# GithinjiHans/LZZX-NeRF

Hardware: AMD Instinct MI355X
Metric: rendered samples/s (512x512 triplane head, max_steps 192) (higher is better)
Workload: dtype f32; 1 GPU; cfg3/cfg4 inference: 512x512 frame, max_steps 192, triplane head (3 hash planes + audio/eye cond + SH4), occupancy=ones; step = ray gen + near/far + march/head/composite + blend; rays_per_rank=262144, parallelism=single GPU, mode=fused

## Files before the change

lzzx_nerf_amd/csrc/lz_frame.hip:

```cpp
#include <stdlib.h>

#include <mutex>

#include "lz_march.h"
#include "lz_head_slice.h"
#include "lz_head_f16_slice.h"
#include "lz_head_f16w_slice.h"

#ifndef LZF_WG
#define LZF_WG 1024
#endif
#define LZF_WAVES (LZF_WG / 64)
#define LZF_BINS 256
#define LZF_LUT 256
#define LZF_MARCH_PROBES 2
#define LZF_Q_HEAD 0
#define LZF_Q_SIZE 1
#define LZF_DONE 3
#define LZF_SAMPLES 5
#define LZF_ITER 6
#define LZF_ROWS 72
#define LZF_P_HEAD 8
#define LZF_P_SIZE 9
#define LZF_CEFF 10
// ... 223 lines not shown
        slot[SF_R * ns + sl] = image[(size_t)ray * 3];
        slot[SF_G * ns + sl] = image[(size_t)ray * 3 + 1];
        slot[SF_B * ns + sl] = image[(size_t)ray * 3 + 2];
        slot[SF_A0 * ns + sl] = LZF_OUT(O, amb0_sum)[ray];
        slot[SF_A1 * ns + sl] = LZF_OUT(O, amb1_sum)[ray];
        slot[SF_U * ns + sl] = LZF_OUT(O, unc_sum)[ray];
        sloti[SF_CNT * ns + sl] = (int)LZF_OUT(O, max_steps);
    } else {
#pragma unroll
        for (int f = SF_WS; f <= SF_U; f++) slot[f * ns + sl] = 0.0f;
        sloti[SF_CNT * ns + sl] = 0;
    }
}
enum { LZF_END_BOX = 0, LZF_END_T = 1, LZF_END_CAP = 2 };
__device__ __forceinline__ void lzf_ray_end(const LzfOut& O, bool ph2, int ray, int kind, int composited, int report, float t, float ws, float d,
                                            float r, float g, float b, float a0, float a1, float u) {
    if (__builtin_expect(LZF_OUT(O, cap_mode) != 0, 0)) {
        report = composited;
        if (kind == LZF_END_T) {
            if (LZF_OUT(O, ray_counts)) { report = -composited; LZF_OUT(O, rays_t)[ray] = t; }
            if (!ph2) LZF_OUT(O, ray_last)[ray] = composited - 1;
        } else if (!ph2) {
            LZF_OUT(O, ray_last)[ray] = composited;
            if (kind == LZF_END_CAP) LZF_OUT(O, rays_t)[ray] = t;
        }
    }
    lzf_write_pixel(O, ray, ws, d, r, g, b, a0, a1, u, report);
}

template <int PREC> struct LzfHead;
template <> struct LzfHead<0> {
    using Args = LzHeadArgs; using Ctx = LzHeadCtx; using Out = LzHeadOut;
    static constexpr int LDS_WORDS = LzHeadLds<false>::FLOATS;
    __device__ static __forceinline__ void stage(const Args& P, float* lds, int q, Ctx& c) { lz_head_stage<false>(P, lds, LZF_WG, q, c); }
    __device__ static __forceinline__ LzShPartial sh(const LzfOut& O, const float* slot, int ls, int ns, int q) {
        const int ray = reinterpret_cast<const int*>(slot)[SF_RAY * ns + ls];
        return LzShPartial{ray >= 0 ? LZF_OUT(O, c1sh) + (size_t)ray * LZ_C1_SH_FLOATS + 16 * q : nullptr};
    }
    template <typename ShFn>
    __device__ static __forceinline__ void slice(const Ctx& c, int lane, float x, float y, float z, ShFn f, Out& o) {
        lz_head_slice<false, false, true, true>(c, lane, x, y, z, f, o);
    }
};
template <> struct LzfHead<2> : LzfHead<0> {
    template <typename ShFn>
    __device__ static __forceinline__ void slice(const Ctx& c, int lane, float x, float y, float z, ShFn f, Out& o) {
        lz_head_slice<false, true, true, true>(c, lane, x, y, z, f, o);
    }
};
template <> struct LzfHead<1> {
    using Args = LzHead16Args; using Ctx = LzHead16Ctx; using Out = LzHead16wOut;
    static constexpr int LDS_WORDS = LZ_HEAD16W_LDS_H8 * 4;
    __device__ static __forceinline__ void stage(const Args& P, float* lds, int, Ctx& c) { lz_head16w_stage(P, reinterpret_cast<lz_h8*>(lds), LZF_WG, c); }
    __device__ static __forceinline__ LzShFromSlot16 sh(const LzfOut&, const float* slot, int ls, int ns, int) { return LzShFromSlot16{slot, ls, ns}; }
    template <typename ShFn>
    __device__ static __forceinline__ void slice(const Ctx& c, int lane, float x, float y, float z, ShFn f, Out& o) {
        lz_head16w_slice<true, LZ_F16W_PRIO != 0>(c, lane, x, y, z, f, o);
    }
};

template <int PREC, int S, int ROWS>
__global__ void __launch_bounds__(LZF_WG, LZF_WG / 256)
lz_k_frame(typename LzfHead<PREC>::Args P, LzFrameK F) {
    using HD = LzfHead<PREC>;
    static_assert(PREC == 1 ? ROWS == 2 : (ROWS == 1 || S == 1), "slot rows per wave: f16 two; f32 one, or several with one sample per ray and pass");
    constexpr int NS = 16 * ROWS;
    using FL = LzfFields<PREC, S, ROWS>;
    constexpr int NF = FL::COUNT;
    constexpr int SF_X = FL::X, SF_Y = FL::Y, SF_Z = FL::Z, SF_TS = FL::TS, SF_OSIG = FL::OSIG, SF_OR = FL::OR, SF_OG = FL::OG, SF_OB = FL::OB,
                  SF_OA0 = FL::OA0, SF_OA1 = FL::OA1, SF_OU = FL::OU, SF_IT = FL::IT, SF_RD = FL::RD;
    (void)SF_RD; (void)SF_X; (void)SF_Y; (void)SF_Z; (void)SF_TS; (void)SF_IT; (void)SF_OSIG; (void)SF_OR; (void)SF_OG; (void)SF_OB; (void)SF_OA0; (void)SF_OA1; (void)SF_OU;
    constexpr int SLOT_WORDS = LZF_WAVES * NF * NS;
    __shared__ __align__(16) float lds[HD::LDS_WORDS + SLOT_WORDS + 4 + LZF_LUT];
    const int lane = threadIdx.x & 63, wave = threadIdx.x >> 6;
    const int s = (S > 1) ? (lane & (NS - 1)) : (lane & 15), q = lane >> 4;
    const bool slot_lane = lane < NS;
    static_assert(alignof(typename HD::Args) <= 8, "lz_k_frame(Args P, LzFrameK F): F sits at round8(sizeof(Args)) of the kernel-argument segment");
    const LzfOut OUT = lzf_out<sizeof(typename HD::Args)>();
    const bool ph2 = F.phase2 != 0;
    if (ph2 && F.state[LZF_P_SIZE] <= 0) return;
    typename HD::Ctx ctx;
    HD::stage(P, lds, q, ctx);
    float* slot = lds + HD::LDS_WORDS + wave * NF * NS;
    int* sloti = reinterpret_cast<int*>(slot);
    int* wg_stat = reinterpret_cast<int*>(lds + HD::LDS_WORDS + SLOT_WORDS);
    if (lane < NS) sloti[SF_RAY * NS + lane] = -1;
    if (threadIdx.x < 4) wg_stat[threadIdx.x] = 0;
    uint32_t* mlut = reinterpret_cast<uint32_t*>(lds + HD::LDS_WORDS + SLOT_WORDS + 4);
    const bool use_lut = F.H <= LZF_LUT;
    if (use_lut && threadIdx.x < LZF_LUT) mlut[threadIdx.x] = lz_expand_bits(threadIdx.x);
    __syncthreads();
    const int n_queue = F.state[ph2 ? LZF_P_SIZE : LZF_Q_SIZE];
#define q_head (F.state + (ph2 ? LZF_P_HEAD : LZF_Q_HEAD))
    const int cap = ph2 ? F.state[LZF_CEFF] : (F.cap_mode ? (int)F.max_steps : (((int)F.max_steps + S - 1) / S) * S);
#define cnt_base (ph2 ? (int)F.max_steps : 0)
    constexpr bool KREFILL = ROWS < 3;
#define LZF_RF(name) (KREFILL ? LZF_OUT(OUT, name) : F.name)
    LzMarch m;
    bool dry = n_queue <= 0;
    int my_samples = 0, my_slices = 0;

    if constexpr (S > 1) {
        const int j = s % S, lead = s - j;
        for (;;) {
            if constexpr (PREC != 1 || LZ_F16W_PRIO != 0) __builtin_amdgcn_s_setprio(2);
            const bool leader = slot_lane && j == 0;
            int ray = leader ? sloti[SF_RAY * NS + s] : -1;
            int kk = 0;
            for (int attempt = 0; attempt < 4; attempt++) {
                const bool need = leader && ray < 0 && !dry;
                const unsigned long long mask = __ballot(need);
                if (mask) {
                    const int first = __ffsll((long long)mask) - 1, take = __popcll(mask);
                    int base = 0;
                    if (lane == first) base = atomicAdd(q_head, take);
// ... 82 lines not shown
                            if (more && rank >= 0) {
                                const int sl = lead + rank;
                                slot[SF_X * NS + sl] = cell.x; slot[SF_Y * NS + sl] = cell.y; slot[SF_Z * NS + sl] = cell.z;
                                slot[SF_DT * NS + sl] = cell.dt;
                                slot[SF_TS * NS + sl] = cn;
                            }
                            t0 = t_new;
                            more = more && got < want && t0 < far;
                        }
                        if (leader && grp) {
                            kk = got;
                            if (kk == 0) {
                                const int c0 = sloti[SF_CNT * NS + s];
                                lzf_ray_end(OUT, ph2, ray, LZF_END_BOX, c0, c0, t0, slot[SF_WS * NS + s], slot[SF_D * NS + s], slot[SF_R * NS + s], slot[SF_G * NS + s],
                                            slot[SF_B * NS + s], slot[SF_A0 * NS + s], slot[SF_A1 * NS + s], slot[SF_U * NS + s]);
                                my_samples += c0 - cnt_base;
                                ray = -1;
                                sloti[SF_RAY * NS + s] = -1;
                            }
                        }
                    }
                }
                if (!__ballot(leader && ray < 0 && !dry)) break;
            }
            if (leader) sloti[SF_IT * NS + s] = kk;
            if (!__ballot(kk > 0)) {
                if (dry) break;
                continue;
            }
            const int lkk = sloti[SF_IT * NS + lead];
            const bool live = sloti[SF_RAY * NS + lead] >= 0 && j < lkk;
            const float px = live ? slot[SF_X * NS + s] : 0.0f, py = live ? slot[SF_Y * NS + s] : 0.0f, pz = live ? slot[SF_Z * NS + s] : 0.0f;
            typename HD::Out o;
            HD::slice(ctx, lane, px, py, pz, HD::sh(OUT, slot, lead, NS, q), o);
            my_slices += ROWS;
            if constexpr (PREC == 1) {
                const int hh = lane >> 5;
                slot[(SF_OR + hh) * NS + s] = o.a;
                slot[(hh ? SF_OSIG : SF_OB) * NS + s] = hh ? 1.0f - lz_expf(-o.b * slot[SF_DT * NS + s]) : o.b;
                if (hh == 0) { slot[SF_OA0 * NS + s] = o.ambaud; slot[SF_OA1 * NS + s] = o.eyeatt; slot[SF_OU * NS + s] = o.unc; }
            } else if (q == 0) {
                slot[SF_OSIG * NS + s] = 1.0f - lz_expf(-o.sigma * slot[SF_DT * NS + s]);
                slot[SF_OR * NS + s] = o.rgb[0]; slot[SF_OG * NS + s] = o.rgb[1]; slot[SF_OB * NS + s] = o.rgb[2];
                slot[SF_OA0 * NS + s] = o.ambaud; slot[SF_OA1 * NS + s] = o.eyeatt; slot[SF_OU * NS + s] = o.unc;
            }
            __builtin_amdgcn_wave_barrier();
            if (leader && kk > 0) {
                float ws = slot[SF_WS * NS + s], d = slot[SF_D * NS + s], r = slot[SF_R * NS + s], g = slot[SF_G * NS + s], b = slot[SF_B * NS + s];
                float a0 = slot[SF_A0 * NS + s], a1 = slot[SF_A1 * NS + s], u = slot[SF_U * NS + s], t = slot[SF_T * NS + s];
                int step = 0;
                while (step < kk) {
                    const int sl = s + step;
                    const float alpha = slot[SF_OSIG * NS + sl];
                    const float T = 1 - ws;
                    const float w = alpha * T;
                    ws += w;
                    t = slot[SF_TS * NS + sl];
                    d = lz_fmaf(w, t, d);
                    r = lz_fmaf(w, slot[SF_OR * NS + sl], r);
                    g = lz_fmaf(w, slot[SF_OG * NS + sl], g);
                    b = lz_fmaf(w, slot[SF_OB * NS + sl], b);
                    a0 = a0 + slot[SF_OA0 * NS + sl];
                    a1 = a1 + slot[SF_OA1 * NS + sl];
                    u = lz_fmaf(w, slot[SF_OU * NS + sl], u);
                    if (T < F.T_thresh) break;
                    step++;
                }
// ... 61 lines not shown
                        probes++;
                    }
                    if (have) {
                        slot[SF_T * NS + sl] = t;
                        slot[SF_DT * NS + sl] = dt;
                    } else if (t < far) {
                        slot[SF_T * NS + sl] = t;
                        x = y = z = 0.0f;
                    } else {
                        const int c0 = sloti[SF_CNT * NS + sl];
                        lzf_ray_end(OUT, ph2, ray, LZF_END_BOX, c0, c0, t, slot[SF_WS * NS + sl], slot[SF_D * NS + sl], slot[SF_R * NS + sl], slot[SF_G * NS + sl],
                                    slot[SF_B * NS + sl], slot[SF_A0 * NS + sl], slot[SF_A1 * NS + sl], slot[SF_U * NS + sl]);
                        my_samples += c0 - cnt_base;
                        ray = -1;
                        sloti[SF_RAY * NS + sl] = -1;
                        x = y = z = 0.0f;
                    }
                }
                if (!__ballot(slot_lane && ray < 0 && !dry)) break;
            }
            const unsigned long long have_mask = __ballot(have);
            if (!have_mask) {
                if (dry && !__ballot(slot_lane && ray >= 0)) break;
                continue;
            }
            typename HD::Out o;
            if constexpr (PREC == 1) {
                const int rs = lane & 31, hh = lane >> 5;
                auto lo2 = [](float v) -> float {
                    const auto r = __builtin_amdgcn_permlane32_swap(__float_as_uint(v), __float_as_uint(v), false, false);
                    return __uint_as_float(r[0]);
                };
                const float px = lo2(x), py = lo2(y), pz = lo2(z);
                HD::slice(ctx, lane, px, py, pz, HD::sh(OUT, slot, rs, NS, q), o);
                my_slices += 2;
                slot[(SF_OR + hh) * NS + rs] = o.a;
                slot[(hh ? SF_OSIG : SF_OB) * NS + rs] = o.b;
                if (hh == 0) { slot[SF_OA0 * NS + rs] = o.ambaud; slot[SF_OA1 * NS + rs] = o.eyeatt; slot[SF_OU * NS + rs] = o.unc; }
            } else {
#pragma unroll 1
                for (int row = 0; row < ROWS; row++) {
                    if (ROWS > 1 && !((have_mask >> (16 * row)) & 0xffffull)) continue;
                    const int rs = 16 * row + s;
                    const float px = __shfl(x, rs, 64), py = __shfl(y, rs, 64), pz = __shfl(z, rs, 64);
                    HD::slice(ctx, lane, px, py, pz, HD::sh(OUT, slot, rs, NS, q), o);
                    my_slices++;
                    if (ROWS > 1 && q == 0) {
                        slot[SF_OSIG * NS + rs] = o.sigma;
                        slot[SF_OR * NS + rs] = o.rgb[0]; slot[SF_OG * NS + rs] = o.rgb[1]; slot[SF_OB * NS + rs] = o.rgb[2];
                        slot[SF_OA0 * NS + rs] = o.ambaud; slot[SF_OA1 * NS + rs] = o.eyeatt; slot[SF_OU * NS + rs] = o.unc;
                    }
                }
            }
            __builtin_amdgcn_wave_barrier();
            if (have) {
                float sg, c0, c1, c2, am0, am1, un;
                if constexpr (PREC != 1) { sg = o.sigma; c0 = o.rgb[0]; c1 = o.rgb[1]; c2 = o.rgb[2]; am0 = o.ambaud; am1 = o.eyeatt; un = o.unc; }
                if (ROWS > 1) {
                    sg = slot[SF_OSIG * NS + sl];
                    c0 = slot[SF_OR * NS + sl]; c1 = slot[SF_OG * NS + sl]; c2 = slot[SF_OB * NS + sl];
                    am0 = slot[SF_OA0 * NS + sl]; am1 = slot[SF_OA1 * NS + sl]; un = slot[SF_OU * NS + sl];
                }
                const float dt = slot[SF_DT * NS + sl];
                float ws = slot[SF_WS * NS + sl];
                const float alpha = 1.0f - lz_expf(-sg * dt);
                const float T = 1 - ws;
                const float w = alpha * T;
                ws += w;
                const float t = slot[SF_T * NS + sl] + dt;
                const float d = lz_fmaf(w, t, slot[SF_D * NS + sl]);
                const float r = lz_fmaf(w, c0, slot[SF_R * NS + sl]);
                const float g = lz_fmaf(w, c1, slot[SF_G * NS + sl]);
                const float b = lz_fmaf(w, c2, slot[SF_B * NS + sl]);
                const float a0 = slot[SF_A0 * NS + sl] + am0;
                const float a1 = slot[SF_A1 * NS + sl] + am1;
                const float u = lz_fmaf(w, un, slot[SF_U * NS + sl]);
                const int cnt = sloti[SF_CNT * NS + sl] + 1;
                if (T < F.T_thresh || cnt >= cap) {
// ... 478 lines not shown
```

lzzx_nerf_amd/csrc/lz_head.hip:

```cpp
#include "lz_head_slice.h"

extern "C" uint32_t lz_head_packed_size(void) { return (uint32_t)LZ_HEAD_PACKED_FLOATS; }

__device__ __forceinline__ int lz_chained(int slot, int K) {
    const int t = slot >> 4, r = (slot & 15) >> 2, q = slot & 3;
    const int f = 16 * t + 4 * q + r;
    return f < K ? f : -1;
}

struct LzPackArgs {
    const float* w[LZ_L_COUNT];
    int nout[LZ_L_COUNT];
    int ld[LZ_L_COUNT];
    const float *eye1, *col1, *unc1;
    int has_eye, has_ind;
};

__device__ __forceinline__ int lz_pack_kf(int layer, int slot, const LzPackArgs& a) {
    switch (layer) {
        case LZ_L_A1: case LZ_L_E1: case LZ_L_U1: return slot < 36 ? slot : -1;
        case LZ_L_A2: case LZ_L_S2: case LZ_L_S3: return lz_chained(slot, 64);
        case LZ_L_S1:
            if (slot < 36) return slot;
            if (slot < 68) return 36 + lz_chained(slot - 36, 32);
// ... 78 lines not shown
        if (kf >= 0 && srow >= 0 && a.w[layer]) v = a.w[layer][(size_t)srow * a.ld[layer] + kf];
        packed[(size_t)gid * 4 + j] = (_Float16)v;
    }
}

extern "C" int lz_head_pack_weights_bwd_f16(const float* aud0, const float* aud1, const float* eye0, const float* sig0, const float* sig1,
                                            const float* sig2, const float* col0, int has_eye, int has_ind, void* packed_bwd16,
                                            lz_stream_t stream) {
    LZ_REQUIRE(aud0 && aud1 && sig0 && sig1 && sig2 && col0 && packed_bwd16, LZ_ERR_BAD_ARGUMENT, "head_pack_weights_bwd_f16: null weight");
    LZ_REQUIRE(!has_eye || eye0, LZ_ERR_BAD_ARGUMENT, "head_pack_weights_bwd_f16: eye weights required when has_eye");
    LzPackArgs a;
    const float* w[LZ_L_COUNT] = {aud0, aud1, eye0, sig0, sig1, sig2, col0, nullptr};
    const int nout[LZ_L_COUNT] = {64, 32, 16, 64, 64, 65, 64, 32};
    const int ld[LZ_L_COUNT] = {36, 64, 36, 68 + (has_eye ? 1 : 0), 64, 64, 80 + (has_ind ? 4 : 0), 36};
    for (int i = 0; i < LZ_L_COUNT; i++) { a.w[i] = w[i]; a.nout[i] = nout[i]; a.ld[i] = ld[i]; }
    a.eye1 = a.col1 = a.unc1 = nullptr;
    a.has_eye = has_eye; a.has_ind = has_ind;
    hipLaunchKernelGGL(lz_k_head_pack_bwd_f16, dim3(lz_div_up((uint64_t)LZ_BFRAGS * 64, 256)), dim3(256), 0, lz_st(stream), a,
                       reinterpret_cast<_Float16*>(packed_bwd16));
    LZ_CHECK_LAUNCH("head_pack_weights_bwd_f16");
    return LZ_OK;
}

#define LZ_WG 1024
#define LZ_WG_SAMPLES (LZ_WG / 64 * LZ_T * 16)

__device__ unsigned long long lz_head_probe[2];

template <bool TRAIN_UNC, bool FOLD = false>
__global__ void __launch_bounds__(LZ_WG, LZ_WG / 256)
lz_k_triplane_head(LzHeadArgs P, const float* __restrict__ xyzs, const float* __restrict__ dirs, uint32_t M,
                   const int* __restrict__ count, float* __restrict__ sigmas, float* __restrict__ rgbs,
                   float* __restrict__ amb_aud, float* __restrict__ amb_eye, float* __restrict__ unc_out) {
    __shared__ float wl[LzHeadLds<TRAIN_UNC>::FLOATS];
    uint32_t Meff = M;
    if (count) {
        const int c = *count;
        Meff = c < 0 ? 0u : ((uint32_t)c < M ? (uint32_t)c : M);
    }
    const uint32_t n_slices = (Meff + LZ_T * 16 - 1) / (LZ_T * 16);
    const uint32_t slice_lo = (uint32_t)(((uint64_t)n_slices * blockIdx.x) / gridDim.x);
    const uint32_t slice_hi = (uint32_t)(((uint64_t)n_slices * (blockIdx.x + 1)) / gridDim.x);
    if (slice_lo >= slice_hi) return;
    const bool probe = blockIdx.x == 0 && threadIdx.x == 0;
    unsigned long long probe_c = 0, probe_w = 0;
    if (probe) { probe_c = clock64(); probe_w = wall_clock64(); }

    const int lane = threadIdx.x & 63;
    const int s = lane & 15, q = lane >> 4;
    LzHeadCtx ctx;
    lz_head_stage<TRAIN_UNC>(P, wl, LZ_WG, q, ctx);
    __syncthreads();

    int* queue = reinterpret_cast<int*>(wl + LzHeadLds<TRAIN_UNC>::TAB) + LZ_LVTAB_QUEUE;
    for (;;) {
        int slice = 0;
        if (lane == 0) slice = atomicAdd(queue, 1);
        slice = __builtin_amdgcn_readfirstlane(slice);
        if (slice_lo + (uint32_t)slice >= slice_hi) {
            if (probe) { lz_head_probe[0] = clock64() - probe_c; lz_head_probe[1] = wall_clock64() - probe_w; }
            break;
        }
        const uint32_t base = (slice_lo + (uint32_t)slice) * (LZ_T * 16);
        uint32_t m = base + s;
        if (m >= Meff) m = Meff - 1;
        const float px = xyzs[(size_t)m * 3], py = xyzs[(size_t)m * 3 + 1], pz = xyzs[(size_t)m * 3 + 2];
        LzHeadOut o;
        lz_head_slice<TRAIN_UNC, FOLD>(ctx, lane, px, py, pz,
                                 lz_sh_from_dir([&](float& dx, float& dy, float& dz) { dx = dirs[(size_t)m * 3]; dy = dirs[(size_t)m * 3 + 1]; dz = dirs[(size_t)m * 3 + 2]; }), o);
        if (q == 0 && base + s < Meff) {
            sigmas[m] = o.sigma;
            rgbs[(size_t)m * 3] = o.rgb[0]; rgbs[(size_t)m * 3 + 1] = o.rgb[1]; rgbs[(size_t)m * 3 + 2] = o.rgb[2];
            amb_aud[m] = o.ambaud;
            if (amb_eye) amb_eye[m] = o.eyeatt;
            unc_out[m] = o.unc;
        }
    }
}

int lz_head_forward_f16_impl(const lz_head_params* p, const float* xyzs, const float* dirs, uint32_t M, const int32_t* count, float* sigmas,
                             float* rgbs, float* amb_aud, float* amb_eye, float* unc, hipStream_t st);

extern "C" int lz_debug_head_clocks(uint64_t* out2) {
    LZ_REQUIRE(out2, LZ_ERR_BAD_ARGUMENT, "debug_head_clocks: null");
// ... 44 lines not shown
```

lzzx_nerf_amd/csrc/lz_head_layers.h:

```cpp
#ifndef LZ_HEAD_LAYERS_H
#define LZ_HEAD_LAYERS_H
#include "lz_common.h"
#include "lzzx_detmath.h"

typedef float lz_f4 __attribute__((ext_vector_type(4)));

enum { LZ_L_A1 = 0, LZ_L_A2, LZ_L_E1, LZ_L_S1, LZ_L_S2, LZ_L_S3, LZ_L_C1, LZ_L_U1, LZ_L_COUNT };
constexpr int LZ_KS[LZ_L_COUNT] = {   9, 16,  9, 18, 16, 16, 21,  9 };
constexpr int LZ_NT[LZ_L_COUNT] = {   4,  2,  1,  4,  4,  4,  4,  2 };
constexpr int lz_frag_base(int layer) {
    int b = 0;
    for (int i = 0; i < layer; i++) b += LZ_KS[i] * LZ_NT[i];
    return b;
}
constexpr int lz_kt(int layer) { return (LZ_KS[layer] + 3) / 4; }
constexpr int lz_bfrag_base(int layer) {
    int b = 0;
    for (int i = 0; i < layer; i++) b += i == LZ_L_U1 ? 0 : lz_kt(i) * LZ_NT[i];
    return b;
}
constexpr int LZ_BFRAGS = lz_bfrag_base(LZ_L_COUNT);
constexpr int LZ_FRAGS_INFER = lz_frag_base(LZ_L_U1);
constexpr int LZ_FRAGS_ALL = lz_frag_base(LZ_L_COUNT);
constexpr int LZ_WV_C2 = 0, LZ_WV_SIG = 192, LZ_WV_E2 = 256, LZ_WV_U2 = 272, LZ_WV_FLOATS = 320;
static_assert(LZ_FRAGS_ALL * 64 + LZ_WV_FLOATS == LZ_HEAD_PACKED_FLOATS, "packed size mismatch with the header");


struct LzHeadArgs {
    const float* emb[3];
    const int* offsets;
    const float* packed;
    const float* enc_a;
    const float* ind_code;
    const float* eye;
    float bound;
    float scale[12];
    uint32_t res[12];
    int testing;
};

template <int LAYER, int T, int K0, int K1>
__device__ __forceinline__ void lz_layer_ks(const float* __restrict__ wl, int lane, const float (&b)[T][LZ_KS[LAYER]],
                                            lz_f4 (&acc)[LZ_NT[LAYER]][T]) {
    constexpr int NT = LZ_NT[LAYER];
    static_assert(0 <= K0 && K0 <= K1 && K1 <= LZ_KS[LAYER], "k-step range");
    const float* frag = wl + lz_frag_base(LAYER) * 64 + lane;
#pragma unroll
    for (int ks = K0; ks < K1; ks++) {
        float a[NT];
#pragma unroll
        for (int ft = 0; ft < NT; ft++) a[ft] = frag[(ks * NT + ft) * 64];
#pragma unroll
        for (int ft = 0; ft < NT; ft++)
#pragma unroll
            for (int j = 0; j < T; j++) acc[ft][j] = __builtin_amdgcn_mfma_f32_16x16x4f32(a[ft], b[j][ks], acc[ft][j], 0, 0, 0);
    }
}
template <int LAYER, int T>
__device__ __forceinline__ void lz_layer(const float* __restrict__ wl, int lane, const float (&b)[T][LZ_KS[LAYER]],
                                         lz_f4 (&acc)[LZ_NT[LAYER]][T]) {
    lz_layer_ks<LAYER, T, 0, LZ_KS[LAYER]>(wl, lane, b, acc);
}

__device__ __forceinline__ float lz_relu(float v) { return v > 0.0f ? v : 0.0f; }

template <int NTILE>
__device__ __forceinline__ float lz_lane_dot(const float* __restrict__ wrow, int q, const float (&x)[4 * NTILE]) {
    float acc = 0.0f;
#pragma unroll
    for (int t = 0; t < NTILE; t++)
#pragma unroll
        for (int r = 0; r < 4; r++) acc = lz_fmaf(wrow[16 * t + 4 * q + r], x[4 * t + r], acc);
    acc += __shfl_xor(acc, 16, 64);
    acc += __shfl_xor(acc, 32, 64);
    return acc;
}

#endif
```

lzzx_nerf_amd/csrc/lz_head_slice.h:

```cpp
#ifndef LZ_HEAD_SLICE_H
#define LZ_HEAD_SLICE_H
#include "lz_common.h"
#include "lzzx_detmath.h"
#include "lzzx_sh_eval.h"
#include "lz_head_gather.h"
#include "lz_head_layers.h"

#define LZ_T 1

struct LzHeadCtx {
    const float* wl;
    const int* tab;
    const float* lenca;
    const float* emb[3];
    float bound, two_bound, eye_v, indq;
    const float* lind;
    bool has_eye, has_ind;
};

struct LzHeadOut {
    float sigma, rgb[3], ambaud, eyeatt, unc;
};

template <bool TRAIN_UNC>
struct LzHeadLds {
    static constexpr int NFRAG = TRAIN_UNC ? LZ_FRAGS_ALL : LZ_FRAGS_INFER;
    static constexpr int WV = NFRAG * 64, TAB = WV + LZ_WV_FLOATS, FLOATS = TAB + LZ_LVTAB_WORDS;
};

template <bool TRAIN_UNC>
__device__ __forceinline__ void lz_head_stage(const LzHeadArgs& P, float* wl, uint32_t n_threads, int q, LzHeadCtx& hc) {
    using L = LzHeadLds<TRAIN_UNC>;
    const float4* src = reinterpret_cast<const float4*>(P.packed);
    float4* dst = reinterpret_cast<float4*>(wl);
    for (uint32_t i = threadIdx.x; i < (uint32_t)L::NFRAG * 16; i += n_threads) dst[i] = src[i];
    if (threadIdx.x < LZ_WV_FLOATS) wl[L::WV + threadIdx.x] = P.packed[LZ_FRAGS_ALL * 64 + threadIdx.x];
    int* tab = reinterpret_cast<int*>(wl + L::TAB);
    lz_level_table_fill(tab, P.offsets, P.scale, P.res);
    if (threadIdx.x < 32) wl[L::TAB + LZ_LVTAB_ENCA + threadIdx.x] = P.enc_a[threadIdx.x];
    hc.wl = wl;
    hc.tab = tab;
    hc.lenca = wl + L::TAB + LZ_LVTAB_ENCA;
    hc.emb[0] = P.emb[0]; hc.emb[1] = P.emb[1]; hc.emb[2] = P.emb[2];
    hc.bound = P.bound;
    hc.two_bound = 2.0f * P.bound;
    hc.has_eye = P.eye != nullptr;
    hc.eye_v = hc.has_eye ? P.eye[0] : 0.0f;
    hc.indq = P.ind_code ? P.ind_code[q] : 0.0f;
    hc.has_ind = P.ind_code != nullptr;
    if (threadIdx.x < 4) wl[L::TAB + LZ_LVTAB_IND + threadIdx.x] = P.ind_code ? P.ind_code[threadIdx.x] : 0.0f;
    hc.lind = wl + L::TAB + LZ_LVTAB_IND;
}

template <typename DirFn>
struct LzShFromDir {
    DirFn dirfn;
    float o[16];
    static constexpr bool C1_PARTIAL = false;
    __device__ __forceinline__ explicit LzShFromDir(DirFn f) : dirfn(f) {}
    __device__ __forceinline__ void issue(int) {}
    __device__ __forceinline__ void prepare() {
        float dx, dy, dz;
        dirfn(dx, dy, dz);
        lz_sh_eval(dx, dy, dz, 4, o, nullptr, nullptr, nullptr);
    }
    __device__ __forceinline__ float comp_iq(int i, int q) const {
        return q == 0 ? o[4 * i] : (q == 1 ? o[4 * i + 1] : (q == 2 ? o[4 * i + 2] : o[4 * i + 3]));
    }
    __device__ __forceinline__ float comp_qj(int q, int j) const {
        return q == 0 ? o[j] : (q == 1 ? o[4 + j] : (q == 2 ? o[8 + j] : o[12 + j]));
    }
};
template <typename DirFn>
__device__ __forceinline__ LzShFromDir<DirFn> lz_sh_from_dir(DirFn f) { return LzShFromDir<DirFn>(f); }

constexpr int LZ_C1_SH_KS = 4;
constexpr int LZ_C1_SH_FLOATS = 64;
template <typename ShFn>
__device__ __forceinline__ void lz_c1_sh_partial(const float* __restrict__ wl, int lane, ShFn& sh, lz_f4 (&acc)[4][1]) {
    const int q = lane >> 4;
    float b[1][LZ_KS[LZ_L_C1]];
    sh.prepare();
#pragma unroll
    for (int i = 0; i < LZ_KS[LZ_L_C1]; i++) b[0][i] = i < LZ_C1_SH_KS ? sh.comp_iq(i, q) : 0.0f;
#pragma unroll
    for (int ft = 0; ft < 4; ft++) acc[ft][0] = lz_f4{0, 0, 0, 0};
    lz_layer_ks<LZ_L_C1, 1, 0, LZ_C1_SH_KS>(wl, lane, b, acc);
}
struct LzShPartial {
    static constexpr bool C1_PARTIAL = true;
    const float* row;
    lz_f4 p[4];
    __device__ __forceinline__ void issue(int) {
#pragma unroll
        for (int ft = 0; ft < 4; ft++) p[ft] = row ? *reinterpret_cast<const lz_f4*>(row + 4 * ft) : lz_f4{0, 0, 0, 0};
    }
    __device__ __forceinline__ lz_f4 part(int ft) const { return p[ft]; }
};

template <bool TRAIN_UNC, bool FOLD = false, bool IN_RANGE = false, bool YIELD = false, typename ShFn>
__device__ __forceinline__ void lz_head_slice(const LzHeadCtx& hc, int lane, float px, float py, float pz, ShFn shfn, LzHeadOut& out) {
    static_assert(!(TRAIN_UNC && FOLD), "the folded colour net is an inference arrangement");
    constexpr int WV = LzHeadLds<TRAIN_UNC>::WV;
    const int q = lane >> 4;
    float encx[LZ_T][9];
    lz_head_gather<IN_RANGE, LZ_GATHER_PACK32, YIELD, true>(hc.emb, hc.tab, px, py, pz, q, hc.bound, hc.two_bound, encx[0]);
    __builtin_amdgcn_sched_barrier(0);

    float att[LZ_T][8];
    {
        lz_f4 acc1[4][LZ_T];
#pragma unroll
        for (int ft = 0; ft < 4; ft++)
#pragma unroll
            for (int j = 0; j < LZ_T; j++) acc1[ft][j] = lz_f4{0, 0, 0, 0};
        lz_layer<LZ_L_A1, LZ_T>(hc.wl, lane, encx, acc1);
        float b2[LZ_T][16];
#pragma unroll
        for (int j = 0; j < LZ_T; j++)
#pragma unroll
            for (int ft = 0; ft < 4; ft++)
#pragma unroll
                for (int r = 0; r < 4; r++) b2[j][4 * ft + r] = lz_relu(acc1[ft][j][r]);
        lz_f4 acc2[2][LZ_T];
#pragma unroll
        for (int ft = 0; ft < 2; ft++)
#pragma unroll
            for (int j = 0; j < LZ_T; j++) acc2[ft][j] = lz_f4{0, 0, 0, 0};
        lz_layer<LZ_L_A2, LZ_T>(hc.wl, lane, b2, acc2);
#pragma unroll
        for (int j = 0; j < LZ_T; j++)
#pragma unroll
            for (int ft = 0; ft < 2; ft++)
#pragma unroll
                for (int r = 0; r < 4; r++) att[j][4 * ft + r] = acc2[ft][j][r];
    }
    float ambaud[LZ_T];
#pragma unroll
    for (int j = 0; j < LZ_T; j++) {
        float acc = 0.0f;
#pragma unroll
        for (int k = 0; k < 8; k++) acc = lz_fmaf(att[j][k], att[j][k], acc);
        acc += __shfl_xor(acc, 16, 64);
        acc += __shfl_xor(acc, 32, 64);
        ambaud[j] = sqrtf(acc);
    }
    float eyeatt[LZ_T];
#pragma unroll
    for (int j = 0; j < LZ_T; j++) eyeatt[j] = 0.0f;
    if (hc.has_eye) {
        lz_f4 acce[1][LZ_T];
#pragma unroll
        for (int j = 0; j < LZ_T; j++) acce[0][j] = lz_f4{0, 0, 0, 0};
        lz_layer<LZ_L_E1, LZ_T>(hc.wl, lane, encx, acce);
        float be[LZ_T][4];
#pragma unroll
        for (int j = 0; j < LZ_T; j++)
#pragma unroll
            for (int r = 0; r < 4; r++) be[j][r] = lz_relu(acce[0][j][r]);
#pragma unroll
        for (int j = 0; j < LZ_T; j++) eyeatt[j] = lz_sigmoidf(lz_lane_dot<1>(hc.wl + WV + LZ_WV_E2, q, be[j]));
    }
    float uncv[LZ_T];
    if constexpr (TRAIN_UNC) {
        lz_f4 accu[2][LZ_T];
#pragma unroll
        for (int ft = 0; ft < 2; ft++)
#pragma unroll
            for (int j = 0; j < LZ_T; j++) accu[ft][j] = lz_f4{0, 0, 0, 0};
        lz_layer<LZ_L_U1, LZ_T>(hc.wl, lane, encx, accu);
        float bu[LZ_T][8];
#pragma unroll
        for (int j = 0; j < LZ_T; j++)
#pragma unroll
            for (int ft = 0; ft < 2; ft++)
#pragma unroll
                for (int r = 0; r < 4; r++) bu[j][4 * ft + r] = lz_relu(accu[ft][j][r]);
#pragma unroll
        for (int j = 0; j < LZ_T; j++) uncv[j] = lz_softplusf(lz_lane_dot<2>(hc.wl + WV + LZ_WV_U2, q, bu[j]));
    } else {
#pragma unroll
        for (int j = 0; j < LZ_T; j++) uncv[j] = lz_softplusf(0.0f);
    }
    float geo[LZ_T][16];
    float sig_pre[LZ_T];
    {
        float b1[LZ_T][18];
#pragma unroll
        for (int j = 0; j < LZ_T; j++) {
#pragma unroll
            for (int i = 0; i < 9; i++) b1[j][i] = encx[j][i];
#pragma unroll
            for (int t = 0; t < 2; t++)
#pragma unroll
                for (int r = 0; r < 4; r++) b1[j][9 + 4 * t + r] = hc.lenca[16 * t + 4 * q + r] * att[j][4 * t + r];
            b1[j][17] = 0.0f;
        }
        lz_f4 acc1[4][LZ_T];
#pragma unroll
        for (int ft = 0; ft < 4; ft++)
#pragma unroll
            for (int j = 0; j < LZ_T; j++) acc1[ft][j] = lz_f4{0, 0, 0, 0};
        lz_layer_ks<LZ_L_S1, LZ_T, 0, 17>(hc.wl, lane, b1, acc1);
        if (hc.has_eye) {
            const float* w68 = hc.wl + (lz_frag_base(LZ_L_S1) + 17 * LZ_NT[LZ_L_S1]) * 64 + 4 * q;
#pragma unroll
            for (int j = 0; j < LZ_T; j++) {
                const float e = hc.eye_v * eyeatt[j];
#pragma unroll
                for (int ft = 0; ft < 4; ft++) {
                    const lz_f4 w = *reinterpret_cast<const lz_f4*>(w68 + 64 * ft);
#pragma unroll
                    for (int r = 0; r < 4; r++) acc1[ft][j][r] = lz_fmaf(w[r], e, acc1[ft][j][r]);
                }
            }
        }
        float b2[LZ_T][16];
#pragma unroll
        for (int j = 0; j < LZ_T; j++)
#pragma unroll
            for (int ft = 0; ft < 4; ft++)
#pragma unroll
                for (int r = 0; r < 4; r++) b2[j][4 * ft + r] = lz_relu(acc1[ft][j][r]);
        shfn.issue(q);
        lz_f4 acc2[4][LZ_T];
#pragma unroll
        for (int ft = 0; ft < 4; ft++)
#pragma unroll
            for (int j = 0; j < LZ_T; j++) acc2[ft][j] = lz_f4{0, 0, 0, 0};
        lz_layer<LZ_L_S2, LZ_T>(hc.wl, lane, b2, acc2);
        float b3[LZ_T][16];
#pragma unroll
        for (int j = 0; j < LZ_T; j++)
#pragma unroll
            for (int ft = 0; ft < 4; ft++)
#pragma unroll
                for (int r = 0; r < 4; r++) b3[j][4 * ft + r] = lz_relu(acc2[ft][j][r]);
        if constexpr (FOLD) {
#pragma unroll
            for (int j = 0; j < LZ_T; j++)
#pragma unroll
                for (int k = 0; k < 16; k++) geo[j][k] = b3[j][k];
        } else {
            lz_f4 acc3[4][LZ_T];
#pragma unroll
            for (int ft = 0; ft < 4; ft++)
#pragma unroll
                for (int j = 0; j < LZ_T; j++) acc3[ft][j] = lz_f4{0, 0, 0, 0};
            lz_layer<LZ_L_S3, LZ_T>(hc.wl, lane, b3, acc3);
#pragma unroll
            for (int j = 0; j < LZ_T; j++)
#pragma unroll
                for (int ft = 0; ft < 4; ft++)
#pragma unroll
                    for (int r = 0; r < 4; r++) geo[j][4 * ft + r] = acc3[ft][j][r];
        }
#pragma unroll
        for (int j = 0; j < LZ_T; j++) sig_pre[j] = lz_lane_dot<4>(hc.wl + WV + LZ_WV_SIG, q, b3[j]);
    }
    float rgb[LZ_T][3];
    {
        constexpr bool IND_VALU = !FOLD;
        float b1[LZ_T][21];
        lz_f4 acc1[4][LZ_T];
#pragma unroll
        for (int j = 0; j < LZ_T; j++) {
            if constexpr (ShFn::C1_PARTIAL) {
#pragma unroll
                for (int i = 0; i < LZ_C1_SH_KS; i++) b1[j][i] = 0.0f;
#pragma unroll
                for (int ft = 0; ft < 4; ft++) acc1[ft][j] = shfn.part(ft);
            } else {
                shfn.prepare();
#pragma unroll
                for (int i = 0; i < 4; i++) b1[j][i] = shfn.comp_iq(i, q);
#pragma unroll
                for (int ft = 0; ft < 4; ft++) acc1[ft][j] = lz_f4{0, 0, 0, 0};
            }
#pragma unroll
            for (int k = 0; k < 16; k++) b1[j][4 + k] = geo[j][k];
            b1[j][20] = IND_VALU ? 0.0f : hc.indq;
        }
        lz_layer_ks<LZ_L_C1, LZ_T, ShFn::C1_PARTIAL ? LZ_C1_SH_KS : 0, LZ_KS[LZ_L_C1] - (IND_VALU ? 1 : 0)>(hc.wl, lane, b1, acc1);
        if (IND_VALU && hc.has_ind) {
            const float* w80 = hc.wl + (lz_frag_base(LZ_L_C1) + 20 * LZ_NT[LZ_L_C1]) * 64 + 4 * q;
            const lz_f4 ind = *reinterpret_cast<const lz_f4*>(hc.lind);
#pragma unroll
            for (int j = 0; j < LZ_T; j++)
#pragma unroll
                for (int k = 0; k < 4; k++)
#pragma unroll
                    for (int ft = 0; ft < 4; ft++) {
                        const lz_f4 w = *reinterpret_cast<const lz_f4*>(w80 + 64 * ft + 16 * k);
#pragma unroll
                        for (int r = 0; r < 4; r++) acc1[ft][j][r] = lz_fmaf(w[r], ind[k], acc1[ft][j][r]);
                    }
        }
        float b2[LZ_T][16];
#pragma unroll
        for (int j = 0; j < LZ_T; j++)
#pragma unroll
            for (int ft = 0; ft < 4; ft++)
#pragma unroll
                for (int r = 0; r < 4; r++) b2[j][4 * ft + r] = lz_relu(acc1[ft][j][r]);
#pragma unroll
        for (int j = 0; j < LZ_T; j++) {
            float d[3];
#pragma unroll
            for (int c = 0; c < 3; c++) d[c] = lz_lane_dot<4>(hc.wl + WV + LZ_WV_C2 + 64 * c, q, b2[j]);
            const float arg = q == 0 ? -d[0] : (q == 1 ? -d[1] : (q == 2 ? -d[2] : sig_pre[j]));
            const float e = lz_expf(arg);
            const float v = q == 3 ? e : (1.0f / (1.0f + e)) * 1.002f - 0.001f;
            const int s0 = lane & 15;
#pragma unroll
            for (int c = 0; c < 3; c++) rgb[j][c] = __shfl(v, s0 + 16 * c, 64);
            sig_pre[j] = __shfl(v, s0 + 48, 64);
        }
    }
    out.sigma = sig_pre[0];
    out.rgb[0] = rgb[0][0]; out.rgb[1] = rgb[0][1]; out.rgb[2] = rgb[0][2];
    out.ambaud = ambaud[0];
    out.eyeatt = eyeatt[0];
    out.unc = uncv[0];
}
#endif
```

Baseline: 2.799 billion samples/s.

## Stage head weights k-step-major in LDS and prefetch next MFMA fragment

Adds a k-step-major LDS weight layout so each lane pulls all NT output-tile weights for one k-step with a single vector load. A new layer routine prefetches the next k-step (or the first fragment of the next layer) while the current MFMAs issue, with scheduling barriers to interleave LDS reads and MFMAs. The frame kernel uses this for the S==1 refill paths and the standalone head kernel always does. The per-step path keeps the planar layout. The cost is extra live registers and a more complex staging transpose, which may lower occupancy.

```diff
diff --git a/lzzx_nerf_amd/csrc/lz_frame.hip b/lzzx_nerf_amd/csrc/lz_frame.hip
--- a/lzzx_nerf_amd/csrc/lz_frame.hip
+++ b/lzzx_nerf_amd/csrc/lz_frame.hip
@@ -279,28 +279,32 @@
 template <> struct LzfHead<0> {
     using Args = LzHeadArgs; using Ctx = LzHeadCtx; using Out = LzHeadOut;
     static constexpr int LDS_WORDS = LzHeadLds<false>::FLOATS;
-    __device__ static __forceinline__ void stage(const Args& P, float* lds, int q, Ctx& c) { lz_head_stage<false>(P, lds, LZF_WG, q, c); }
+    template <bool KSMAJOR>
+    __device__ static __forceinline__ void stage(const Args& P, float* lds, int q, Ctx& c) {
+        lz_head_stage<false, KSMAJOR ? LZ_W_KSMAJOR : LZ_W_PLANAR>(P, lds, LZF_WG, q, c);
+    }
     __device__ static __forceinline__ LzShPartial sh(const LzfOut& O, const float* slot, int ls, int ns, int q) {
         const int ray = reinterpret_cast<const int*>(slot)[SF_RAY * ns + ls];
         return LzShPartial{ray >= 0 ? LZF_OUT(O, c1sh) + (size_t)ray * LZ_C1_SH_FLOATS + 16 * q : nullptr};
     }
-    template <typename ShFn>
+    template <bool AHEAD, typename ShFn>
     __device__ static __forceinline__ void slice(const Ctx& c, int lane, float x, float y, float z, ShFn f, Out& o) {
-        lz_head_slice<false, false, true, true>(c, lane, x, y, z, f, o);
+        lz_head_slice<false, false, true, true, AHEAD>(c, lane, x, y, z, f, o);
     }
 };
 template <> struct LzfHead<2> : LzfHead<0> {
-    template <typename ShFn>
+    template <bool AHEAD, typename ShFn>
     __device__ static __forceinline__ void slice(const Ctx& c, int lane, float x, float y, float z, ShFn f, Out& o) {
-        lz_head_slice<false, true, true, true>(c, lane, x, y, z, f, o);
+        lz_head_slice<false, true, true, true, AHEAD>(c, lane, x, y, z, f, o);
     }
 };
 template <> struct LzfHead<1> {
     using Args = LzHead16Args; using Ctx = LzHead16Ctx; using Out = LzHead16wOut;
     static constexpr int LDS_WORDS = LZ_HEAD16W_LDS_H8 * 4;
+    template <bool>
     __device__ static __forceinline__ void stage(const Args& P, float* lds, int, Ctx& c) { lz_head16w_stage(P, reinterpret_cast<lz_h8*>(lds), LZF_WG, c); }
     __device__ static __forceinline__ LzShFromSlot16 sh(const LzfOut&, const float* slot, int ls, int ns, int) { return LzShFromSlot16{slot, ls, ns}; }
-    template <typename ShFn>
+    template <bool, typename ShFn>
     __device__ static __forceinline__ void slice(const Ctx& c, int lane, float x, float y, float z, ShFn f, Out& o) {
         lz_head16w_slice<true, LZ_F16W_PRIO != 0>(c, lane, x, y, z, f, o);
     }
@@ -327,7 +331,7 @@
     const bool ph2 = F.phase2 != 0;
     if (ph2 && F.state[LZF_P_SIZE] <= 0) return;
     typename HD::Ctx ctx;
-    HD::stage(P, lds, q, ctx);
+    HD::template stage<S == 1>(P, lds, q, ctx);
     float* slot = lds + HD::LDS_WORDS + wave * NF * NS;
     int* sloti = reinterpret_cast<int*>(slot);
     int* wg_stat = reinterpret_cast<int*>(lds + HD::LDS_WORDS + SLOT_WORDS);
@@ -476,7 +480,7 @@
             const bool live = sloti[SF_RAY * NS + lead] >= 0 && j < lkk;
             const float px = live ? slot[SF_X * NS + s] : 0.0f, py = live ? slot[SF_Y * NS + s] : 0.0f, pz = live ? slot[SF_Z * NS + s] : 0.0f;
             typename HD::Out o;
-            HD::slice(ctx, lane, px, py, pz, HD::sh(OUT, slot, lead, NS, q), o);
+            HD::template slice<false>(ctx, lane, px, py, pz, HD::sh(OUT, slot, lead, NS, q), o);
             my_slices += ROWS;
             if constexpr (PREC == 1) {
                 const int hh = lane >> 5;
@@ -604,7 +608,7 @@
                     return __uint_as_float(r[0]);
                 };
                 const float px = lo2(x), py = lo2(y), pz = lo2(z);
-                HD::slice(ctx, lane, px, py, pz, HD::sh(OUT, slot, rs, NS, q), o);
+                HD::template slice<true>(ctx, lane, px, py, pz, HD::sh(OUT, slot, rs, NS, q), o);
                 my_slices += 2;
                 slot[(SF_OR + hh) * NS + rs] = o.a;
                 slot[(hh ? SF_OSIG : SF_OB) * NS + rs] = o.b;
@@ -615,7 +619,7 @@
                     if (ROWS > 1 && !((have_mask >> (16 * row)) & 0xffffull)) continue;
                     const int rs = 16 * row + s;
                     const float px = __shfl(x, rs, 64), py = __shfl(y, rs, 64), pz = __shfl(z, rs, 64);
-                    HD::slice(ctx, lane, px, py, pz, HD::sh(OUT, slot, rs, NS, q), o);
+                    HD::template slice<true>(ctx, lane, px, py, pz, HD::sh(OUT, slot, rs, NS, q), o);
                     my_slices++;
                     if (ROWS > 1 && q == 0) {
                         slot[SF_OSIG * NS + rs] = o.sigma;
diff --git a/lzzx_nerf_amd/csrc/lz_head.hip b/lzzx_nerf_amd/csrc/lz_head.hip
--- a/lzzx_nerf_amd/csrc/lz_head.hip
+++ b/lzzx_nerf_amd/csrc/lz_head.hip
@@ -134,7 +134,7 @@
 lz_k_triplane_head(LzHeadArgs P, const float* __restrict__ xyzs, const float* __restrict__ dirs, uint32_t M,
                    const int* __restrict__ count, float* __restrict__ sigmas, float* __restrict__ rgbs,
                    float* __restrict__ amb_aud, float* __restrict__ amb_eye, float* __restrict__ unc_out) {
-    __shared__ float wl[LzHeadLds<TRAIN_UNC>::FLOATS];
+    __shared__ __align__(16) float wl[LzHeadLds<TRAIN_UNC>::FLOATS];
     uint32_t Meff = M;
     if (count) {
         const int c = *count;
@@ -151,7 +151,7 @@
     const int lane = threadIdx.x & 63;
     const int s = lane & 15, q = lane >> 4;
     LzHeadCtx ctx;
-    lz_head_stage<TRAIN_UNC>(P, wl, LZ_WG, q, ctx);
+    lz_head_stage<TRAIN_UNC, LZ_W_KSMAJOR>(P, wl, LZ_WG, q, ctx);
     __syncthreads();
 
     int* queue = reinterpret_cast<int*>(wl + LzHeadLds<TRAIN_UNC>::TAB) + LZ_LVTAB_QUEUE;
diff --git a/lzzx_nerf_amd/csrc/lz_head_layers.h b/lzzx_nerf_amd/csrc/lz_head_layers.h
--- a/lzzx_nerf_amd/csrc/lz_head_layers.h
+++ b/lzzx_nerf_amd/csrc/lz_head_layers.h
@@ -39,7 +39,28 @@
     int testing;
 };
 
-template <int LAYER, int T, int K0, int K1>
+enum { LZ_W_PLANAR = 0, LZ_W_KSMAJOR = 1 };
+template <int LAYER>
+__device__ __forceinline__ constexpr int lz_w_at(int ks, int lane, int ft) {
+    return (lz_frag_base(LAYER) + ks * LZ_NT[LAYER]) * 64 + lane * LZ_NT[LAYER] + ft;
+}
+template <int NT> struct LzWFrag { float v[NT]; };
+template <int LAYER>
+__device__ __forceinline__ LzWFrag<LZ_NT[LAYER]> lz_wfetch(const float* __restrict__ wl, int lane, int ks) {
+    constexpr int NT = LZ_NT[LAYER];
+    LzWFrag<NT> a;
+    if constexpr (NT > 1) {
+        typedef float vec_t __attribute__((ext_vector_type(NT)));
+        const vec_t w = *reinterpret_cast<const vec_t*>(wl + lz_w_at<LAYER>(ks, lane, 0));
+#pragma unroll
+        for (int ft = 0; ft < NT; ft++) a.v[ft] = w[ft];
+    } else {
+        a.v[0] = wl[lz_w_at<LAYER>(ks, lane, 0)];
+    }
+    return a;
+}
+
+template <int LAYER, int T, int K0, int K1, int LAYOUT = LZ_W_PLANAR>
 __device__ __forceinline__ void lz_layer_ks(const float* __restrict__ wl, int lane, const float (&b)[T][LZ_KS[LAYER]],
                                             lz_f4 (&acc)[LZ_NT[LAYER]][T]) {
     constexpr int NT = LZ_NT[LAYER];
@@ -48,13 +69,51 @@
 #pragma unroll
     for (int ks = K0; ks < K1; ks++) {
         float a[NT];
+        if constexpr (LAYOUT == LZ_W_KSMAJOR) {
+            const LzWFrag<NT> w = lz_wfetch<LAYER>(wl, lane, ks);
 #pragma unroll
-        for (int ft = 0; ft < NT; ft++) a[ft] = frag[(ks * NT + ft) * 64];
+            for (int ft = 0; ft < NT; ft++) a[ft] = w.v[ft];
+        } else {
+#pragma unroll
+            for (int ft = 0; ft < NT; ft++) a[ft] = frag[(ks * NT + ft) * 64];
+        }
 #pragma unroll
         for (int ft = 0; ft < NT; ft++)
 #pragma unroll
             for (int j = 0; j < T; j++) acc[ft][j] = __builtin_amdgcn_mfma_f32_16x16x4f32(a[ft], b[j][ks], acc[ft][j], 0, 0, 0);
     }
+}
+constexpr int lz_nt_or1(int layer) { return layer < 0 ? 1 : LZ_NT[layer]; }
+template <bool AHEAD, int LAYER, int T, int K0, int K1, int NEXT = -1, int NEXT_K = 0, int NEXT2 = -1, int NEXT2_K = 0>
+__device__ __forceinline__ LzWFrag<lz_nt_or1(NEXT)> lz_layer_ks_ahead(const float* __restrict__ wl, int lane, const float (&b)[T][LZ_KS[LAYER]],
+                                                                     lz_f4 (&acc)[LZ_NT[LAYER]][T], LzWFrag<LZ_NT[LAYER]> a,
+                                                                     LzWFrag<lz_nt_or1(NEXT2)>* next2 = nullptr) {
+    constexpr int NT = LZ_NT[LAYER];
+    static_assert(0 <= K0 && K0 < K1 && K1 <= LZ_KS[LAYER], "k-step range");
+    LzWFrag<lz_nt_or1(NEXT)> next = {};
+    if constexpr (!AHEAD) {
+        lz_layer_ks<LAYER, T, K0, K1, LZ_W_PLANAR>(wl, lane, b, acc);
+        return next;
+    }
+#pragma unroll
+    for (int ks = K0; ks < K1; ks++) {
+        LzWFrag<NT> ahead = a;
+        if (ks + 1 < K1) ahead = lz_wfetch<LAYER>(wl, lane, ks + 1);
+        else {
+            if constexpr (NEXT >= 0) next = lz_wfetch<NEXT>(wl, lane, NEXT_K);
+            if constexpr (NEXT2 >= 0) *next2 = lz_wfetch<NEXT2>(wl, lane, NEXT2_K);
+        }
+#pragma unroll
+        for (int ft = 0; ft < NT; ft++)
+#pragma unroll
+            for (int j = 0; j < T; j++) acc[ft][j] = __builtin_amdgcn_mfma_f32_16x16x4f32(a.v[ft], b[j][ks], acc[ft][j], 0, 0, 0);
+        if (ks + 1 < K1 || NEXT >= 0) __builtin_amdgcn_sched_group_barrier(0x100 , 1, 0);
+        if (ks + 1 == K1 && NEXT2 >= 0) __builtin_amdgcn_sched_group_barrier(0x100, 1, 0);
+        __builtin_amdgcn_sched_group_barrier(0x8 , NT * T, 0);
+        a = ahead;
+    }
+    __builtin_amdgcn_sched_barrier(0);
+    return next;
 }
 template <int LAYER, int T>
 __device__ __forceinline__ void lz_layer(const float* __restrict__ wl, int lane, const float (&b)[T][LZ_KS[LAYER]],
diff --git a/lzzx_nerf_amd/csrc/lz_head_slice.h b/lzzx_nerf_amd/csrc/lz_head_slice.h
--- a/lzzx_nerf_amd/csrc/lz_head_slice.h
+++ b/lzzx_nerf_amd/csrc/lz_head_slice.h
@@ -28,12 +28,35 @@
     static constexpr int WV = NFRAG * 64, TAB = WV + LZ_WV_FLOATS, FLOATS = TAB + LZ_LVTAB_WORDS;
 };
 
-template <bool TRAIN_UNC>
+template <int LAYER>
+__device__ __forceinline__ void lz_head_stage_ksmajor(const float* __restrict__ packed, float* wl, uint32_t n_threads) {
+    constexpr int NT = LZ_NT[LAYER], BASE = lz_frag_base(LAYER);
+    const float4* src = reinterpret_cast<const float4*>(packed) + BASE * 16;
+    for (uint32_t i = threadIdx.x; i < (uint32_t)(LZ_KS[LAYER] * NT * 16); i += n_threads) {
+        const float4 v = src[i];
+        const int f = (int)(i >> 4), l0 = (int)(i & 15) * 4;
+        float* d = wl + lz_w_at<LAYER>(f / NT, l0, f % NT);
+        d[0] = v.x; d[NT] = v.y; d[2 * NT] = v.z; d[3 * NT] = v.w;
+    }
+}
+template <bool TRAIN_UNC, int LAYER = 0>
+__device__ __forceinline__ void lz_head_stage_ksmajor_all(const float* __restrict__ packed, float* wl, uint32_t n_threads) {
+    if constexpr (LAYER < (TRAIN_UNC ? LZ_L_COUNT : LZ_L_U1)) {
+        lz_head_stage_ksmajor<LAYER>(packed, wl, n_threads);
+        lz_head_stage_ksmajor_all<TRAIN_UNC, LAYER + 1>(packed, wl, n_threads);
+    }
+}
+
+template <bool TRAIN_UNC, int LAYOUT = LZ_W_PLANAR>
 __device__ __forceinline__ void lz_head_stage(const LzHeadArgs& P, float* wl, uint32_t n_threads, int q, LzHeadCtx& hc) {
     using L = LzHeadLds<TRAIN_UNC>;
-    const float4* src = reinterpret_cast<const float4*>(P.packed);
-    float4* dst = reinterpret_cast<float4*>(wl);
-    for (uint32_t i = threadIdx.x; i < (uint32_t)L::NFRAG * 16; i += n_threads) dst[i] = src[i];
+    if constexpr (LAYOUT == LZ_W_KSMAJOR) {
+        lz_head_stage_ksmajor_all<TRAIN_UNC>(P.packed, wl, n_threads);
+    } else {
+        const float4* src = reinterpret_cast<const float4*>(P.packed);
+        float4* dst = reinterpret_cast<float4*>(wl);
+        for (uint32_t i = threadIdx.x; i < (uint32_t)L::NFRAG * 16; i += n_threads) dst[i] = src[i];
+    }
     if (threadIdx.x < LZ_WV_FLOATS) wl[L::WV + threadIdx.x] = P.packed[LZ_FRAGS_ALL * 64 + threadIdx.x];
     int* tab = reinterpret_cast<int*>(wl + L::TAB);
     lz_level_table_fill(tab, P.offsets, P.scale, P.res);
@@ -98,23 +121,27 @@
     __device__ __forceinline__ lz_f4 part(int ft) const { return p[ft]; }
 };
 
-template <bool TRAIN_UNC, bool FOLD = false, bool IN_RANGE = false, bool YIELD = false, typename ShFn>
+template <bool TRAIN_UNC, bool FOLD = false, bool IN_RANGE = false, bool YIELD = false, bool AHEAD = true, typename ShFn>
 __device__ __forceinline__ void lz_head_slice(const LzHeadCtx& hc, int lane, float px, float py, float pz, ShFn shfn, LzHeadOut& out) {
     static_assert(!(TRAIN_UNC && FOLD), "the folded colour net is an inference arrangement");
     constexpr int WV = LzHeadLds<TRAIN_UNC>::WV;
     const int q = lane >> 4;
     float encx[LZ_T][9];
     lz_head_gather<IN_RANGE, LZ_GATHER_PACK32, YIELD, true>(hc.emb, hc.tab, px, py, pz, q, hc.bound, hc.two_bound, encx[0]);
+    LzWFrag<4> w_a1 = {};
+    if constexpr (AHEAD) w_a1 = lz_wfetch<LZ_L_A1>(hc.wl, lane, 0);
     __builtin_amdgcn_sched_barrier(0);
 
     float att[LZ_T][8];
+    LzWFrag<1> w_e1;
+    LzWFrag<4> w_s1;
     {
         lz_f4 acc1[4][LZ_T];
 #pragma unroll
         for (int ft = 0; ft < 4; ft++)
 #pragma unroll
             for (int j = 0; j < LZ_T; j++) acc1[ft][j] = lz_f4{0, 0, 0, 0};
-        lz_layer<LZ_L_A1, LZ_T>(hc.wl, lane, encx, acc1);
+        const LzWFrag<2> w_a2 = lz_layer_ks_ahead<AHEAD, LZ_L_A1, LZ_T, 0, LZ_KS[LZ_L_A1], LZ_L_A2, 0>(hc.wl, lane, encx, acc1, w_a1);
         float b2[LZ_T][16];
 #pragma unroll
         for (int j = 0; j < LZ_T; j++)
@@ -127,7 +154,7 @@
         for (int ft = 0; ft < 2; ft++)
 #pragma unroll
             for (int j = 0; j < LZ_T; j++) acc2[ft][j] = lz_f4{0, 0, 0, 0};
-        lz_layer<LZ_L_A2, LZ_T>(hc.wl, lane, b2, acc2);
+        w_e1 = lz_layer_ks_ahead<AHEAD, LZ_L_A2, LZ_T, 0, LZ_KS[LZ_L_A2], LZ_L_E1, 0, LZ_L_S1, 0>(hc.wl, lane, b2, acc2, w_a2, &w_s1);
 #pragma unroll
         for (int j = 0; j < LZ_T; j++)
 #pragma unroll
@@ -148,11 +175,12 @@
     float eyeatt[LZ_T];
 #pragma unroll
     for (int j = 0; j < LZ_T; j++) eyeatt[j] = 0.0f;
+    if constexpr (AHEAD) asm volatile("" : "+v"(w_e1.v[0]));
     if (hc.has_eye) {
         lz_f4 acce[1][LZ_T];
 #pragma unroll
         for (int j = 0; j < LZ_T; j++) acce[0][j] = lz_f4{0, 0, 0, 0};
-        lz_layer<LZ_L_E1, LZ_T>(hc.wl, lane, encx, acce);
+        lz_layer_ks_ahead<AHEAD, LZ_L_E1, LZ_T, 0, LZ_KS[LZ_L_E1]>(hc.wl, lane, encx, acce, w_e1);
         float be[LZ_T][4];
 #pragma unroll
         for (int j = 0; j < LZ_T; j++)
@@ -168,7 +196,7 @@
         for (int ft = 0; ft < 2; ft++)
 #pragma unroll
             for (int j = 0; j < LZ_T; j++) accu[ft][j] = lz_f4{0, 0, 0, 0};
-        lz_layer<LZ_L_U1, LZ_T>(hc.wl, lane, encx, accu);
+        lz_layer_ks_ahead<AHEAD, LZ_L_U1, LZ_T, 0, LZ_KS[LZ_L_U1]>(hc.wl, lane, encx, accu, lz_wfetch<LZ_L_U1>(hc.wl, lane, 0));
         float bu[LZ_T][8];
 #pragma unroll
         for (int j = 0; j < LZ_T; j++)
@@ -184,6 +212,7 @@
     }
     float geo[LZ_T][16];
     float sig_pre[LZ_T];
+    LzWFrag<4> w_c1;
     {
         float b1[LZ_T][18];
 #pragma unroll
@@ -201,17 +230,21 @@
         for (int ft = 0; ft < 4; ft++)
 #pragma unroll
             for (int j = 0; j < LZ_T; j++) acc1[ft][j] = lz_f4{0, 0, 0, 0};
-        lz_layer_ks<LZ_L_S1, LZ_T, 0, 17>(hc.wl, lane, b1, acc1);
+        if constexpr (AHEAD) __builtin_amdgcn_sched_barrier(0);
+        const LzWFrag<4> w_s2 = lz_layer_ks_ahead<AHEAD, LZ_L_S1, LZ_T, 0, 17, LZ_L_S2, 0>(hc.wl, lane, b1, acc1, w_s1);
         if (hc.has_eye) {
-            const float* w68 = hc.wl + (lz_frag_base(LZ_L_S1) + 17 * LZ_NT[LZ_L_S1]) * 64 + 4 * q;
+            const float* w68 = AHEAD ? hc.wl + lz_w_at<LZ_L_S1>(17, 4 * q, 0) : hc.wl + (lz_frag_base(LZ_L_S1) + 17 * LZ_NT[LZ_L_S1]) * 64 + 4 * q;
 #pragma unroll
             for (int j = 0; j < LZ_T; j++) {
                 const float e = hc.eye_v * eyeatt[j];
 #pragma unroll
-                for (int ft = 0; ft < 4; ft++) {
-                    const lz_f4 w = *reinterpret_cast<const lz_f4*>(w68 + 64 * ft);
-#pragma unroll
-                    for (int r = 0; r < 4; r++) acc1[ft][j][r] = lz_fmaf(w[r], e, acc1[ft][j][r]);
+                for (int u = 0; u < 4; u++) {
+                    const lz_f4 w = *reinterpret_cast<const lz_f4*>(w68 + (AHEAD ? 4 : 64) * u);
+#pragma unroll
+                    for (int v = 0; v < 4; v++) {
+                        const int ft = AHEAD ? v : u, r = AHEAD ? u : v;
+                        acc1[ft][j][r] = lz_fmaf(w[v], e, acc1[ft][j][r]);
+                    }
                 }
             }
         }
@@ -228,7 +261,8 @@
         for (int ft = 0; ft < 4; ft++)
 #pragma unroll
             for (int j = 0; j < LZ_T; j++) acc2[ft][j] = lz_f4{0, 0, 0, 0};
-        lz_layer<LZ_L_S2, LZ_T>(hc.wl, lane, b2, acc2);
+        constexpr int C1_K0 = ShFn::C1_PARTIAL ? LZ_C1_SH_KS : 0;
+        const LzWFrag<4> w_s3 = lz_layer_ks_ahead<AHEAD, LZ_L_S2, LZ_T, 0, LZ_KS[LZ_L_S2], FOLD ? LZ_L_C1 : LZ_L_S3, FOLD ? C1_K0 : 0>(hc.wl, lane, b2, acc2, w_s2);
         float b3[LZ_T][16];
 #pragma unroll
         for (int j = 0; j < LZ_T; j++)
@@ -241,13 +275,14 @@
             for (int j = 0; j < LZ_T; j++)
 #pragma unroll
                 for (int k = 0; k < 16; k++) geo[j][k] = b3[j][k];
+            w_c1 = w_s3;
         } else {
             lz_f4 acc3[4][LZ_T];
 #pragma unroll
             for (int ft = 0; ft < 4; ft++)
 #pragma unroll
                 for (int j = 0; j < LZ_T; j++) acc3[ft][j] = lz_f4{0, 0, 0, 0};
-            lz_layer<LZ_L_S3, LZ_T>(hc.wl, lane, b3, acc3);
+            w_c1 = lz_layer_ks_ahead<AHEAD, LZ_L_S3, LZ_T, 0, LZ_KS[LZ_L_S3], LZ_L_C1, C1_K0>(hc.wl, lane, b3, acc3, w_s3);
 #pragma unroll
             for (int j = 0; j < LZ_T; j++)
 #pragma unroll
@@ -281,19 +316,23 @@
             for (int k = 0; k < 16; k++) b1[j][4 + k] = geo[j][k];
             b1[j][20] = IND_VALU ? 0.0f : hc.indq;
         }
-        lz_layer_ks<LZ_L_C1, LZ_T, ShFn::C1_PARTIAL ? LZ_C1_SH_KS : 0, LZ_KS[LZ_L_C1] - (IND_VALU ? 1 : 0)>(hc.wl, lane, b1, acc1);
+        if constexpr (AHEAD) __builtin_amdgcn_sched_barrier(0);
+        lz_layer_ks_ahead<AHEAD, LZ_L_C1, LZ_T, ShFn::C1_PARTIAL ? LZ_C1_SH_KS : 0, LZ_KS[LZ_L_C1] - (IND_VALU ? 1 : 0)>(hc.wl, lane, b1, acc1, w_c1);
         if (IND_VALU && hc.has_ind) {
-            const float* w80 = hc.wl + (lz_frag_base(LZ_L_C1) + 20 * LZ_NT[LZ_L_C1]) * 64 + 4 * q;
+            const float* w80 = AHEAD ? hc.wl + lz_w_at<LZ_L_C1>(20, 4 * q, 0) : hc.wl + (lz_frag_base(LZ_L_C1) + 20 * LZ_NT[LZ_L_C1]) * 64 + 4 * q;
             const lz_f4 ind = *reinterpret_cast<const lz_f4*>(hc.lind);
 #pragma unroll
             for (int j = 0; j < LZ_T; j++)
 #pragma unroll
                 for (int k = 0; k < 4; k++)
 #pragma unroll
-                    for (int ft = 0; ft < 4; ft++) {
-                        const lz_f4 w = *reinterpret_cast<const lz_f4*>(w80 + 64 * ft + 16 * k);
-#pragma unroll
-                        for (int r = 0; r < 4; r++) acc1[ft][j][r] = lz_fmaf(w[r], ind[k], acc1[ft][j][r]);
+                    for (int u = 0; u < 4; u++) {
+                        const lz_f4 w = *reinterpret_cast<const lz_f4*>(w80 + (AHEAD ? 64 * k + 4 * u : 64 * u + 16 * k));
+#pragma unroll
+                        for (int v = 0; v < 4; v++) {
+                            const int ft = AHEAD ? v : u, r = AHEAD ? u : v;
+                            acc1[ft][j][r] = lz_fmaf(w[v], ind[k], acc1[ft][j][r]);
+                        }
                     }
         }
         float b2[LZ_T][16];
```

Result: slower. 2.756 billion samples/s (-1.5%).
